# vision-agh/apse_uav

Hardware: AMD Instinct MI355X
Metric: 4K UAV frames/sec (whole node) (higher is better)
Workload: dtype f32

## Files before the change

### apse_uav_amd/csrc/conv_winograd.hip

```cpp
#include "apse_common.h"

namespace {
constexpr int WTR = 16, WTC = 4;
constexpr int WT = WTR * WTC;
constexpr int WN = 64;
constexpr int KC = 8;
constexpr int NTHR = 512;
constexpr int G_U = 1, G_ROWS = 2, G_V = 3;
constexpr int SLICE_F = 16 * WT * KC;
constexpr size_t WINO_LDS = (size_t)2 * 2 * SLICE_F * sizeof(float);
static_assert(WN == WT, "V and U slices share one size");
static_assert((size_t)16 * WT * 32 * sizeof(float) <= WINO_LDS, "epilogue chunk must fit the staging LDS");
}

__global__ __launch_bounds__(NTHR) void conv_winograd_f32(const ConvParams p) {
    extern __shared__ __attribute__((aligned(16))) char smem[];
    float* Vs = reinterpret_cast<float*>(smem);
    float* Us = Vs + 2 * SLICE_F;
    float* Cs = reinterpret_cast<float*>(smem);

    const int tid = threadIdx.x;
    const int lane = tid & 63, wave = __builtin_amdgcn_readfirstlane(tid >> 6);
    const int fr = lane & 31, fh = lane >> 5;

    const int tiles_y = (p.OH + 2 * WTR - 1) / (2 * WTR), tiles_x = (p.OW + 2 * WTC - 1) / (2 * WTC);
    const int nblk = p.Cout / WN;
    const int nwg = p.B * tiles_y * tiles_x * nblk;
    int bid;
    {
        const int wg = blockIdx.x;
        const int q = nwg >> 3, r = nwg & 7, xcd = wg & 7, idx = wg >> 3;
        bid = (xcd < r ? xcd * (q + 1) : r * (q + 1) + (xcd - r) * q) + idx;
    }
    const int nb = bid % nblk;
    int rest = bid / nblk;
    const int bx = rest % tiles_x; rest /= tiles_x;
    const int by = rest % tiles_y;
    const int b = rest / tiles_y;
    const int oy0 = by * 2 * WTR, ox0 = bx * 2 * WTC, n0 = nb * WN;
    const int C = 1 << p.cin_log2;
    const int nsteps = C / KC;

    const int cg = tid & 1, t = (tid >> 1) & (WT - 1), ti = wave >> 1;
    const int ra = ti == 0 ? 0 : (ti == 2 ? 2 : 1);
    const int rb = ti == 0 ? 2 : (ti == 1 ? 2 : (ti == 2 ? 1 : 3));
    const float sgn = ti == 1 ? 1.f : -1.f;
    const int iy_a = oy0 + 2 * (t / WTC) - 1 + ra, iy_b = oy0 + 2 * (t / WTC) - 1 + rb;
    const int ix0 = ox0 + 2 * (t % WTC) - 1;
    const __amdgpu_buffer_rsrc_t xrsrc =
        __builtin_amdgcn_make_buffer_rsrc(const_cast<float*>(p.x), 0, (int)((((unsigned)(p.B * p.H * p.W)) << p.cin_log2) * 4u), 0x00020000);
    const __amdgpu_buffer_rsrc_t xnone = __builtin_amdgcn_make_buffer_rsrc(const_cast<float*>(p.x), 0, 0, 0x00020000);
    unsigned xoff[2][4];
#pragma unroll
    for (int r = 0; r < 2; ++r) {
        const int iy = r ? iy_b : iy_a;
#pragma unroll
        for (int c = 0; c < 4; ++c) {
            const int ix = ix0 + c;
            const bool in = (unsigned)iy < (unsigned)p.H && (unsigned)ix < (unsigned)p.W;
            xoff[r][c] = in ? ((((unsigned)((b * p.H + iy) * p.W + ix)) << p.cin_log2) + (unsigned)(cg * 4)) * 4u : 0x80000000u;
        }
    }
    const __amdgpu_buffer_rsrc_t ursrc =
        __builtin_amdgcn_make_buffer_rsrc(const_cast<float*>(p.wu), 0, (int)((((unsigned)(16 * p.Cout)) << p.cin_log2) * 4u), 0x00020000);
    const unsigned ustep = (unsigned)(16 * p.Cout * KC * 4);
    unsigned uoff[4], ulds[4];
#pragma unroll
    for (int k = 0; k < 4; ++k) {
        const int q = tid + NTHR * k;
        const int xi = q >> 7, co = (q >> 1) & 63, h = q & 1;
        uoff[k] = (unsigned)(((xi * p.Cout + n0 + co) * KC + h * 4) * 4);
        ulds[k] = (unsigned)((xi * WN + co) * KC + ((h ^ ((co >> 3) & 1)) * 4));
    }
    const int vlds = (4 * ti * WT + t) * KC + (cg ^ ((t >> 3) & 1)) * 4;

    f32x4 xr[2][4], ur[4];
    auto fetch_u = [&](int s) {
        const unsigned kb = (unsigned)s * ustep;
#pragma unroll
        for (int k = 0; k < 4; ++k) ur[k] = __builtin_bit_cast(f32x4, __builtin_amdgcn_raw_buffer_load_b128(ursrc, (int)(uoff[k] + kb), 0, 0));
    };
    auto fetch_x = [&](int s) {
        const unsigned kb = (unsigned)(s * KC * 4);
        const __amdgpu_buffer_rsrc_t rs = s < nsteps ? xrsrc : xnone;
#pragma unroll
        for (int r = 0; r < 2; ++r)
#pragma unroll
            for (int c = 0; c < 4; ++c)
                xr[r][c] = __builtin_bit_cast(f32x4, __builtin_amdgcn_raw_buffer_load_b128(rs, (int)(xoff[r][c] + kb), 0, 0));
    };
    auto write_u = [&](int buf) {
#pragma unroll
        for (int k = 0; k < 4; ++k) *reinterpret_cast<f32x4*>(Us + buf * SLICE_F + ulds[k]) = ur[k];
    };
    auto xform_rows = [&]() {
#pragma unroll
        for (int c = 0; c < 4; ++c)
#pragma unroll
            for (int e = 0; e < 4; ++e) xr[0][c][e] = __builtin_fmaf(xr[1][c][e], sgn, xr[0][c][e]);
    };
    auto write_v = [&](int buf) {
        const f32x4 v[4] = {xr[0][0] - xr[0][2], xr[0][1] + xr[0][2], xr[0][2] - xr[0][1], xr[0][1] - xr[0][3]};
#pragma unroll
        for (int j = 0; j < 4; ++j) *reinterpret_cast<f32x4*>(Vs + buf * SLICE_F + vlds + j * WT * KC) = v[j];
    };

    f32x16 acc[2][2][2];
#pragma unroll
    for (int a = 0; a < 2; ++a)
#pragma unroll
        for (int i = 0; i < 2; ++i)
#pragma unroll
            for (int j = 0; j < 2; ++j)
#pragma unroll
                for (int v = 0; v < 16; ++v) acc[a][i][j][v] = 0.f;

    fetch_u(0);
    fetch_x(0);
    write_u(0);
    xform_rows();
    write_v(0);
    __builtin_amdgcn_sched_barrier(0);
    fetch_u(1);
    __builtin_amdgcn_sched_barrier(0);
    fetch_x(1);
    __syncthreads();
    const int fsw = (fh ^ ((fr >> 3) & 1)) * 4;
    const int frag = (2 * wave * WT + fr) * KC + fsw;
    f32x4 af[2][2], bf[2][2];
    auto read_frags = [&](int buf, int a) {
#pragma unroll
        for (int i = 0; i < 2; ++i) af[a][i] = *reinterpret_cast<const f32x4*>(Vs + buf * SLICE_F + frag + (a * WT + 32 * i) * KC);
#pragma unroll
        for (int j = 0; j < 2; ++j) bf[a][j] = *reinterpret_cast<const f32x4*>(Us + buf * SLICE_F + frag + (a * WN + 32 * j) * KC);
    };
    auto mfma_group = [&](int a, int k) {
#pragma unroll
        for (int i = 0; i < 2; ++i)
#pragma unroll
            for (int j = 0; j < 2; ++j)
                acc[a][i][j] = __builtin_amdgcn_mfma_f32_32x32x2f32(af[a][i][k], bf[a][j][k], acc[a][i][j], 0, 0, 0);
    };
    read_frags(0, 0);
    for (int s = 0; s < nsteps; ++s) {
        const int buf = s & 1;
        read_frags(buf, 1);
#pragma unroll
        for (int g = 0; g < 7; ++g) {
            __builtin_amdgcn_sched_barrier(0);
            if (g == G_U) { write_u(buf ^ 1); fetch_u(s + 2); }
            if (g == G_ROWS) xform_rows();
            if (g == G_V) { write_v(buf ^ 1); fetch_x(s + 2); }
            __builtin_amdgcn_sched_barrier(0);
            mfma_group(g >> 2, g & 3);
        }
        __builtin_amdgcn_sched_barrier(0);
        __syncthreads();
        read_frags(buf ^ 1, 0);
        __builtin_amdgcn_sched_barrier(0);
        mfma_group(1, 3);
    }

    const int et = tid >> 3, eg = tid & 7;
    const int oy = oy0 + 2 * (et / WTC), ox = ox0 + 2 * (et % WTC);
    typedef unsigned u32x4_t __attribute__((ext_vector_type(4)));
#pragma unroll
    for (int j = 0; j < 2; ++j) {
#pragma unroll
        for (int a = 0; a < 2; ++a)
#pragma unroll
            for (int i = 0; i < 2; ++i)
#pragma unroll
                for (int v = 0; v < 16; ++v) {
                    const int row = 32 * i + (v & 3) + 8 * (v >> 2) + 4 * fh;
                    Cs[((2 * wave + a) * WT + row) * 32 + fr] = acc[a][i][j][v];
                }
        __syncthreads();
        f32x4 m[16];
#pragma unroll
        for (int k = 0; k < 16; ++k) m[k] = *reinterpret_cast<const f32x4*>(Cs + (k * WT + et) * 32 + eg * 4);
        f32x4 s0[4], s1[4];
#pragma unroll
        for (int c = 0; c < 4; ++c) {
            s0[c] = m[c] + m[4 + c] + m[8 + c];
            s1[c] = m[4 + c] - m[8 + c] - m[12 + c];
        }
        const int co = n0 + 32 * j + 4 * eg;
        const f32x4 bias4 = p.bias ? *reinterpret_cast<const f32x4*>(p.bias + co) : f32x4{0.f, 0.f, 0.f, 0.f};
        f32x4 y[2][2] = {{s0[0] + s0[1] + s0[2], s0[1] - s0[2] - s0[3]}, {s1[0] + s1[1] + s1[2], s1[1] - s1[2] - s1[3]}};
#pragma unroll
        for (int dy = 0; dy < 2; ++dy)
#pragma unroll
            for (int dx = 0; dx < 2; ++dx) {
                f32x4 val = y[dy][dx] + bias4;
                if (p.relu) {
#pragma unroll
                    for (int k = 0; k < 4; ++k) val[k] = apse_relu(val[k]);
                }
                if (oy + dy < p.OH && ox + dx < p.OW)
                    APSE_NT_STORE(val, reinterpret_cast<f32x4*>(p.y + ((size_t)(b * p.OH + oy + dy) * p.OW + ox + dx) * p.y_ld + p.y_coff + co));
            }
        __syncthreads();
    }
}

bool apse_conv_winograd_ok(const ConvParams& p, int max_items) {
    return p.prec == 0 && p.x_st == 0 && p.y_st == 0 && p.KH == 3 && p.KW == 3 && p.stride == 1 && p.pad == 1 && p.out_mode == 0 &&
           p.res_mode == 0 && p.splitk == 1 && p.Cout % WN == 0 && p.cin_log2 >= 3 && p.OH == p.H && p.OW == p.W &&
           (p.y_ld & 3) == 0 && (p.y_coff & 3) == 0 && ((((size_t)max_items * p.H * p.W) << p.cin_log2) * 4 < 0x7fff0000ull);
}

int apse_conv_winograd_blocks(const ConvParams& p) {
    return ((p.OH + 2 * WTR - 1) / (2 * WTR)) * ((p.OW + 2 * WTC - 1) / (2 * WTC)) * (p.Cout / WN);
}

int apse_launch_conv_winograd(const ConvParams& p, hipStream_t s, hipEvent_t ev0, hipEvent_t ev1) {
    if (!p.wu || !apse_conv_winograd_ok(p, p.B) || p.m_count) return APSE_E_INVALID;
    static bool attr_done = false;
    if (!attr_done) {
        hipFuncSetAttribute(reinterpret_cast<const void*>(&conv_winograd_f32), hipFuncAttributeMaxDynamicSharedMemorySize, (int)WINO_LDS);
        attr_done = true;
    }
    const int tiles_y = (p.OH + 2 * WTR - 1) / (2 * WTR), tiles_x = (p.OW + 2 * WTC - 1) / (2 * WTC);
    const int grid = p.B * tiles_y * tiles_x * (p.Cout / WN);
    if (ev0) hipEventRecord(ev0, s);
    hipLaunchKernelGGL(conv_winograd_f32, dim3(grid), dim3(NTHR), WINO_LDS, s, p);
    if (ev1) hipEventRecord(ev1, s);
    return hipGetLastError() == hipSuccess ? APSE_OK : APSE_E_HIP;
}
```

Before: 205.3.

## Stage raw input halo tile in LDS and gather Winograd taps from it

```diff
diff --git a/apse_uav_amd/csrc/conv_winograd.hip b/apse_uav_amd/csrc/conv_winograd.hip
--- a/apse_uav_amd/csrc/conv_winograd.hip
+++ b/apse_uav_amd/csrc/conv_winograd.hip
@@ -6,17 +6,32 @@
 constexpr int WN = 64;
 constexpr int KC = 8;
 constexpr int NTHR = 512;
-constexpr int G_U = 1, G_ROWS = 2, G_V = 3;
+constexpr int G_U = 1, G_TAPS = 0, G_ROWS = 1, G_V = 2, G_RAW = 3;
 constexpr int SLICE_F = 16 * WT * KC;
-constexpr size_t WINO_LDS = (size_t)2 * 2 * SLICE_F * sizeof(float);
+constexpr int PR = 2 * WTR + 2, PC = 2 * WTC + 2;
+constexpr int RAW_PIECES = PR * PC * 2;
+__host__ __device__ constexpr int raw_row(int pr) { return 24 * pr - ((pr & 1) ? 4 : 0) + ((pr & 2) ? 2 : 0); }
+constexpr int RAW_F = (raw_row(PR - 1) + 2 * PC) * 4;
+constexpr size_t WINO_LDS = (size_t)(2 * 2 * SLICE_F + 2 * RAW_F) * sizeof(float);
+static_assert(PC == 10 && KC == 8, "raw_row / raw_piece are laid out for rows of 10 pixels x 2 pieces");
+static_assert(RAW_PIECES <= 2 * NTHR, "at most two raw pieces per thread");
+static_assert(WINO_LDS <= 163840, "one workgroup's LDS");
 static_assert(WN == WT, "V and U slices share one size");
-static_assert((size_t)16 * WT * 32 * sizeof(float) <= WINO_LDS, "epilogue chunk must fit the staging LDS");
+static_assert((size_t)16 * WT * 32 * sizeof(float) <= (size_t)2 * 2 * SLICE_F * sizeof(float), "epilogue chunk must fit the V / U staging");
+
+__device__ __forceinline__ void raw_piece(int q, int& pr, int& pc, int& h) {
+    const int g = q >> 3, k = g % 5, j = (q >> 1) & 3;
+    h = q & 1;
+    pr = 2 * (g / 5) + (k < 4 ? k >> 1 : j >> 1);
+    pc = k < 4 ? 4 * (k & 1) + j : 8 + (j & 1);
+}
 }
 
 __global__ __launch_bounds__(NTHR) void conv_winograd_f32(const ConvParams p) {
     extern __shared__ __attribute__((aligned(16))) char smem[];
     float* Vs = reinterpret_cast<float*>(smem);
     float* Us = Vs + 2 * SLICE_F;
+    float* Raw = Us + 2 * SLICE_F;
     float* Cs = reinterpret_cast<float*>(smem);
 
     const int tid = threadIdx.x;
@@ -45,22 +60,22 @@
     const int ra = ti == 0 ? 0 : (ti == 2 ? 2 : 1);
     const int rb = ti == 0 ? 2 : (ti == 1 ? 2 : (ti == 2 ? 1 : 3));
     const float sgn = ti == 1 ? 1.f : -1.f;
-    const int iy_a = oy0 + 2 * (t / WTC) - 1 + ra, iy_b = oy0 + 2 * (t / WTC) - 1 + rb;
-    const int ix0 = ox0 + 2 * (t % WTC) - 1;
     const __amdgpu_buffer_rsrc_t xrsrc =
         __builtin_amdgcn_make_buffer_rsrc(const_cast<float*>(p.x), 0, (int)((((unsigned)(p.B * p.H * p.W)) << p.cin_log2) * 4u), 0x00020000);
     const __amdgpu_buffer_rsrc_t xnone = __builtin_amdgcn_make_buffer_rsrc(const_cast<float*>(p.x), 0, 0, 0x00020000);
-    unsigned xoff[2][4];
-#pragma unroll
-    for (int r = 0; r < 2; ++r) {
-        const int iy = r ? iy_b : iy_a;
-#pragma unroll
-        for (int c = 0; c < 4; ++c) {
-            const int ix = ix0 + c;
-            const bool in = (unsigned)iy < (unsigned)p.H && (unsigned)ix < (unsigned)p.W;
-            xoff[r][c] = in ? ((((unsigned)((b * p.H + iy) * p.W + ix)) << p.cin_log2) + (unsigned)(cg * 4)) * 4u : 0x80000000u;
-        }
-    }
+    unsigned roff[2];
+    int rlds[2];
+#pragma unroll
+    for (int k = 0; k < 2; ++k) {
+        const int q = tid + NTHR * k;
+        int pr, pc, h;
+        raw_piece(q < RAW_PIECES ? q : tid, pr, pc, h);
+        const int iy = oy0 - 1 + pr, ix = ox0 - 1 + pc;
+        const bool in = q < RAW_PIECES && (unsigned)iy < (unsigned)p.H && (unsigned)ix < (unsigned)p.W;
+        roff[k] = in ? ((((unsigned)((b * p.H + iy) * p.W + ix)) << p.cin_log2) + (unsigned)(h * 4)) * 4u : 0x80000000u;
+        rlds[k] = (raw_row(pr) + 2 * pc + h) * 4;
+    }
+    const int tap_a = (raw_row(2 * (t / WTC) + ra) + 4 * (t % WTC) + cg) * 4, tap_b = (raw_row(2 * (t / WTC) + rb) + 4 * (t % WTC) + cg) * 4;
     const __amdgpu_buffer_rsrc_t ursrc =
         __builtin_amdgcn_make_buffer_rsrc(const_cast<float*>(p.wu), 0, (int)((((unsigned)(16 * p.Cout)) << p.cin_log2) * 4u), 0x00020000);
     const unsigned ustep = (unsigned)(16 * p.Cout * KC * 4);
@@ -74,20 +89,28 @@
     }
     const int vlds = (4 * ti * WT + t) * KC + (cg ^ ((t >> 3) & 1)) * 4;
 
-    f32x4 xr[2][4], ur[4];
+    f32x4 xr[2][4], ur[4], rr[2];
     auto fetch_u = [&](int s) {
         const unsigned kb = (unsigned)s * ustep;
 #pragma unroll
         for (int k = 0; k < 4; ++k) ur[k] = __builtin_bit_cast(f32x4, __builtin_amdgcn_raw_buffer_load_b128(ursrc, (int)(uoff[k] + kb), 0, 0));
     };
-    auto fetch_x = [&](int s) {
+    auto fetch_raw = [&](int s) {
         const unsigned kb = (unsigned)(s * KC * 4);
         const __amdgpu_buffer_rsrc_t rs = s < nsteps ? xrsrc : xnone;
 #pragma unroll
-        for (int r = 0; r < 2; ++r)
-#pragma unroll
-            for (int c = 0; c < 4; ++c)
-                xr[r][c] = __builtin_bit_cast(f32x4, __builtin_amdgcn_raw_buffer_load_b128(rs, (int)(xoff[r][c] + kb), 0, 0));
+        for (int k = 0; k < 2; ++k) rr[k] = __builtin_bit_cast(f32x4, __builtin_amdgcn_raw_buffer_load_b128(rs, (int)(roff[k] + kb), 0, 0));
+    };
+    auto write_raw = [&](int rbuf) {
+#pragma unroll
+        for (int k = 1; k >= 0; --k) *reinterpret_cast<f32x4*>(Raw + rbuf * RAW_F + rlds[k]) = rr[k];
+    };
+    auto read_taps = [&](int rbuf) {
+#pragma unroll
+        for (int c = 0; c < 4; ++c) {
+            xr[0][c] = *reinterpret_cast<const f32x4*>(Raw + rbuf * RAW_F + tap_a + 8 * c);
+            xr[1][c] = *reinterpret_cast<const f32x4*>(Raw + rbuf * RAW_F + tap_b + 8 * c);
+        }
     };
     auto write_u = [&](int buf) {
 #pragma unroll
@@ -116,14 +139,19 @@
                 for (int v = 0; v < 16; ++v) acc[a][i][j][v] = 0.f;
 
     fetch_u(0);
-    fetch_x(0);
+    fetch_raw(0);
     write_u(0);
-    xform_rows();
-    write_v(0);
+    write_raw(0);
     __builtin_amdgcn_sched_barrier(0);
     fetch_u(1);
     __builtin_amdgcn_sched_barrier(0);
-    fetch_x(1);
+    fetch_raw(1);
+    __syncthreads();
+    read_taps(0);
+    xform_rows();
+    write_v(0);
+    write_raw(1);
+    fetch_raw(2);
     __syncthreads();
     const int fsw = (fh ^ ((fr >> 3) & 1)) * 4;
     const int frag = (2 * wave * WT + fr) * KC + fsw;
@@ -149,8 +177,10 @@
         for (int g = 0; g < 7; ++g) {
             __builtin_amdgcn_sched_barrier(0);
             if (g == G_U) { write_u(buf ^ 1); fetch_u(s + 2); }
+            if (g == G_TAPS) read_taps(buf ^ 1);
             if (g == G_ROWS) xform_rows();
-            if (g == G_V) { write_v(buf ^ 1); fetch_x(s + 2); }
+            if (g == G_V) write_v(buf ^ 1);
+            if (g == G_RAW) { write_raw(buf); fetch_raw(s + 3); }
             __builtin_amdgcn_sched_barrier(0);
             mfma_group(g >> 2, g & 3);
         }
```

Result: no change. 207.0, median of 6 (+0.8%).
